# TengdaHan/DPC

Hardware: AMD Instinct MI355X
Metric: clips/sec (train step, B x8x3x5xHxW) (higher is better)
Workload: dtype bf16; 1 GPU; cfg2: resnet18 2d3d, img_dim 128, seq_len 5, num_seq 8, pred_step 3, batch 128/GPU, full train step (fwd+CE/top-k+bwd+all-reduce+Adam); global_batch=128, parallelism=dp1, init=reference init, random, launch=hipGraph replay, streams=2

## Files before the change

### dpc_amd/csrc/bn.hip

```cpp
#include "dpc_rt.h"
#include "../../include/dpc_hip.h"
#include <stdlib.h>

static inline unsigned grid_for(long long n, int block = 256, int cap = 8192) {
    long long g = (n + block - 1) / block;
    if (g < 1) g = 1;
    if (g > cap) g = cap;
    return (unsigned)g;
}

constexpr int FIN_THREADS = 256;
__device__ __forceinline__ void partial_rows_sum(const float* partials, int rows, int C, double& s1, double& s2, double (*red)[4][32]) {
    const int tid = threadIdx.x, q = tid & 7, rl = tid >> 3;
    const int c0 = blockIdx.x * 32 + 4 * q;
    double a[4] = {0.0, 0.0, 0.0, 0.0}, b[4] = {0.0, 0.0, 0.0, 0.0};
    if ((C & 3) == 0 && ((uintptr_t)partials & 15) == 0) {
        if (c0 < C) {
            int r = rl;
            for (; r + 96 < rows; r += 128) {
                f32x4 x[4], y[4];
                DPC_UNROLL
                for (int k = 0; k < 4; ++k) {
                    x[k] = *(const f32x4*)(partials + ((long long)(r + 32 * k) * 2 + 0) * C + c0);
                    y[k] = *(const f32x4*)(partials + ((long long)(r + 32 * k) * 2 + 1) * C + c0);
                }
                DPC_UNROLL
                for (int e = 0; e < 4; ++e) {
                    a[e] += ((double)x[0][e] + (double)x[1][e]) + ((double)x[2][e] + (double)x[3][e]);
                    b[e] += ((double)y[0][e] + (double)y[1][e]) + ((double)y[2][e] + (double)y[3][e]);
                }
            }
            for (; r < rows; r += 32) {
                const f32x4 x = *(const f32x4*)(partials + ((long long)r * 2 + 0) * C + c0);
                const f32x4 y = *(const f32x4*)(partials + ((long long)r * 2 + 1) * C + c0);
                DPC_UNROLL
                for (int e = 0; e < 4; ++e) { a[e] += (double)x[e]; b[e] += (double)y[e]; }
            }
        }
    } else {
        for (int r = rl; r < rows; r += 32)
            DPC_UNROLL
            for (int e = 0; e < 4; ++e)
                if (c0 + e < C) {
                    a[e] += (double)partials[((long long)r * 2 + 0) * C + c0 + e];
                    b[e] += (double)partials[((long long)r * 2 + 1) * C + c0 + e];
                }
    }
    DPC_UNROLL
    for (int m = 8; m < 64; m <<= 1)
        DPC_UNROLL
        for (int e = 0; e < 4; ++e) { a[e] += __shfl_xor(a[e], m); b[e] += __shfl_xor(b[e], m); }
    const int wave = tid >> 6;
    if ((tid & 63) < 8)
        DPC_UNROLL
        for (int e = 0; e < 4; ++e) { red[0][wave][4 * q + e] = a[e]; red[1][wave][4 * q + e] = b[e]; }
    __syncthreads();
    s1 = 0.0; s2 = 0.0;
    if (tid < 32)
        for (int w = 0; w < 4; ++w) { s1 += red[0][w][tid]; s2 += red[1][w][tid]; }
}

__global__ __launch_bounds__(FIN_THREADS) void bn_finalize_kernel(const float* partials, int rows, int C, double count, const float* gamma,
                                   const float* beta, float eps, float* mean, float* invstd, float* scale, float* shift) {
    __shared__ double red[2][4][32];
    const int c = blockIdx.x * 32 + (int)threadIdx.x;
    double s1, s2;
    partial_rows_sum(partials, rows, C, s1, s2, red);
    if (threadIdx.x >= 32 || c >= C) return;
    const double m = s1 / count;
    double var = s2 / count - m * m;
    if (var < 0.0) var = 0.0;
    const double is = 1.0 / sqrt(var + (double)eps);
    mean[c] = (float)m;
    invstd[c] = (float)is;
    const float sc = gamma[c] * (float)is;
    scale[c] = sc;
    shift[c] = beta[c] - (float)m * sc;
}

extern "C" int dpc_bn_finalize(const float* partials, int32_t rows, int32_t C, double count, const float* gamma,
                               const float* beta, float eps, float* mean, float* invstd, float* scale, float* shift,
                               dpc_stream_t stream_) {
    hipStream_t stream = (hipStream_t)stream_;
    if (!partials || rows <= 0 || C <= 0 || count <= 0 || !gamma || !beta || !mean || !invstd || !scale || !shift) return DPC_ERR_ARG;
    DPC_LAUNCH(bn_finalize_kernel, dim3((C + 31) / 32), dim3(FIN_THREADS), stream, partials, rows, C, count, gamma, beta, eps, mean, invstd, scale, shift);
// ... 120 lines not shown
                for (int e = 0; e < E; ++e) {
                    float v = unit_get<T>(xv[u], e) * sc[e] + sh[e];
                    if (res) v += unit_get<T>(rv[u], e) * rs[e] + rb[e];
                    if (relu) v = v > 0.f ? v : 0.f;
                    ov[e] = v;
                }
                const u32x4 o = unit_pack<T>(ov);
                st16<NT>(y, i + u * 256, o);
                if (mask) {
                    DPC_UNROLL
                    for (int e = 0; e < E; ++e) bits |= (unit_get<T>(o, e) > 0.f ? 1u : 0u) << e;
                    mask[i + u * 256] = (uint8_t)bits;
                }
            }
        }
    }
    for (; i < se; i += 256) {
        if (!FIXED) {
            const int c0 = (int)((i * E) % C);
            DPC_UNROLL
            for (int e = 0; e < E; ++e) {
                sc[e] = scale[c0 + e]; sh[e] = shift[c0 + e];
                rs[e] = rscale ? rscale[c0 + e] : 1.f; rb[e] = rscale ? rshift[c0 + e] : 0.f;
            }
        }
        const u32x4 xv = ld16<NT>(x, i);
        u32x4 rv = {0u, 0u, 0u, 0u};
        if (res) rv = ld16<NT>(res, i);
        float ov[E];
        unsigned bits = 0;
        DPC_UNROLL
        for (int e = 0; e < E; ++e) {
            float v = unit_get<T>(xv, e) * sc[e] + sh[e];
            if (res) v += unit_get<T>(rv, e) * rs[e] + rb[e];
            if (relu) v = v > 0.f ? v : 0.f;
            ov[e] = v;
        }
        const u32x4 o = unit_pack<T>(ov);
        st16<NT>(y, i, o);
        if (mask) {
            DPC_UNROLL
            for (int e = 0; e < E; ++e) bits |= (unit_get<T>(o, e) > 0.f ? 1u : 0u) << e;
            mask[i] = (uint8_t)bits;
        }
    }
}

extern "C" int dpc_bn_apply(const void* x, void* y, int32_t dtype, int64_t rows, int32_t C, const float* scale,
                            const float* shift, const void* res, const float* rscale, const float* rshift, int32_t relu,
                            uint8_t* mask, dpc_stream_t stream_) {
    hipStream_t stream = (hipStream_t)stream_;
    if (!x || !y || rows <= 0 || C <= 0 || !scale || !shift) return DPC_ERR_ARG;
    const int E = dtype == DPC_BF16 ? 8 : 4;
    if (C % E) return DPC_ERR_UNSUPPORTED;
    const long long units = rows * C / E;
    const bool fixed = (256 * E) % C == 0;
    static const int rev_on = getenv("DPC_BN_APPLY_REV") ? atoi(getenv("DPC_BN_APPLY_REV")) : 0;
    const int rev = rev_on && bn_streaming(units) ? 1 : 0;
    if (rev && (dtype == DPC_F32 || dtype == DPC_BF16)) dpc_plan_detail("rev");
    if (dtype == DPC_F32) {
        if (fixed) {
            if (bn_streaming(units)) { DPC_LAUNCH((bn_apply_kernel<float, true, true>), dim3(grid_for(units)), dim3(256), stream, (const float*)x, (float*)y, units, C, scale, shift, (const float*)res, rscale, rshift, relu, mask, rev); } else { DPC_LAUNCH((bn_apply_kernel<float, true, false>), dim3(grid_for(units)), dim3(256), stream, (const float*)x, (float*)y, units, C, scale, shift, (const float*)res, rscale, rshift, relu, mask, rev); }
        } else {
            if (bn_streaming(units)) { DPC_LAUNCH((bn_apply_kernel<float, false, true>), dim3(grid_for(units)), dim3(256), stream, (const float*)x, (float*)y, units, C, scale, shift, (const float*)res, rscale, rshift, relu, mask, rev); } else { DPC_LAUNCH((bn_apply_kernel<float, false, false>), dim3(grid_for(units)), dim3(256), stream, (const float*)x, (float*)y, units, C, scale, shift, (const float*)res, rscale, rshift, relu, mask, rev); }
        }
    } else if (dtype == DPC_BF16) {
        if (fixed) {
            const bool nt = bn_streaming(units);
            const int un = nt ? bn_unroll() : bn_small_unroll();
            const unsigned grid = grid_for((units + un - 1) / un, 256, nt ? (un > 1 ? bn_unroll_grid() : 8192) : bn_small_grid(512));
#define DPC_BN_GO(NTV, UV) DPC_LAUNCH((bn_apply_kernel<bf16_t, true, NTV, UV>), dim3(grid), dim3(256), stream, (const bf16_t*)x, (bf16_t*)y, units, C, scale, shift, (const bf16_t*)res, rscale, rshift, relu, mask, rev)
            if (nt) { if (un == 4) DPC_BN_GO(true, 4); else if (un == 2) DPC_BN_GO(true, 2); else DPC_BN_GO(true, 1); }
            else { if (un == 4) DPC_BN_GO(false, 4); else if (un == 2) DPC_BN_GO(false, 2); else DPC_BN_GO(false, 1); }
#undef DPC_BN_GO
        } else {
            if (bn_streaming(units)) { DPC_LAUNCH((bn_apply_kernel<bf16_t, false, true>), dim3(grid_for(units)), dim3(256), stream, (const bf16_t*)x, (bf16_t*)y, units, C, scale, shift, (const bf16_t*)res, rscale, rshift, relu, mask, rev); } else { DPC_LAUNCH((bn_apply_kernel<bf16_t, false, false>), dim3(grid_for(units)), dim3(256), stream, (const bf16_t*)x, (bf16_t*)y, units, C, scale, shift, (const bf16_t*)res, rscale, rshift, relu, mask, rev); }
        }
    } else {
        return DPC_ERR_ARG;
    }
    return dpc_launch_status();
}

template <class T, bool NT, int U = 1>
__global__ __launch_bounds__(256) void bn_bwd_reduce_kernel(const T* dy, const T* y, const uint8_t* mask, const T* x, long long rows, int C,
                                                            const float* mean, const float* invstd, int relu,
                                                            float* partials, long long rows_per_block) {
    constexpr int E = Elt<T>::PER16;
    __shared__ float red[2][256 * E];
    const int upr = C / E;
    const int rpi = 256 / upr;
    const int tid = threadIdx.x;
    const int cu = tid % upr, rr = tid / upr;
    float a1[E], a2[E], mu[E], is[E];
    DPC_UNROLL
    for (int e = 0; e < E; ++e) { a1[e] = 0.f; a2[e] = 0.f; }
    const bool active = rr < rpi;
    if (active) {
        DPC_UNROLL
        for (int e = 0; e < E; ++e) { mu[e] = mean[cu * E + e]; is[e] = invstd[cu * E + e]; }
        const long long r_begin = (long long)blockIdx.x * rows_per_block;
        long long r_end = r_begin + rows_per_block;
        if (r_end > rows) r_end = rows;
        long long r = r_begin + rr;
        if constexpr (U > 1) {
            if (!relu || mask) {
                for (; r + (long long)(U - 1) * rpi < r_end; r += (long long)U * rpi) {
                    u32x4 dv[U], xv[U];
                    unsigned bits[U];
                    DPC_UNROLL
                    for (int u = 0; u < U; ++u) dv[u] = ld16<NT>(dy, (r + (long long)u * rpi) * upr + cu);
                    DPC_UNROLL
                    for (int u = 0; u < U; ++u) xv[u] = ld16<NT>(x, (r + (long long)u * rpi) * upr + cu);
                    DPC_UNROLL
                    for (int u = 0; u < U; ++u) bits[u] = relu ? (unsigned)mask[(r + (long long)u * rpi) * upr + cu] : ~0u;
                    DPC_UNROLL
                    for (int u = 0; u < U; ++u)
                        DPC_UNROLL
                        for (int e = 0; e < E; ++e) {
                            float dz = unit_get<T>(dv[u], e);
                            if (!((bits[u] >> e) & 1u)) dz = 0.f;
                            const float xh = (unit_get<T>(xv[u], e) - mu[e]) * is[e];
                            a1[e] += dz;
                            a2[e] += dz * xh;
                        }
                }
            }
        }
        for (; r < r_end; r += rpi) {
            const long long ui = r * upr + cu;
            const u32x4 dv = ld16<NT>(dy, ui);
            const u32x4 xv = ld16<NT>(x, ui);
            unsigned bits = ~0u;
            if (relu) bits = mask ? (unsigned)mask[ui] : sign_bits<T>(((const u32x4*)y)[ui]);
            DPC_UNROLL
            for (int e = 0; e < E; ++e) {
                float dz = unit_get<T>(dv, e);
                if (!((bits >> e) & 1u)) dz = 0.f;
                const float xh = (unit_get<T>(xv, e) - mu[e]) * is[e];
                a1[e] += dz;
                a2[e] += dz * xh;
            }
        }
    }
    DPC_UNROLL
    for (int e = 0; e < E; ++e) {
        red[0][tid * E + e] = a1[e];
        red[1][tid * E + e] = a2[e];
    }
    __syncthreads();
    if (tid < C) {
        const int cu2 = tid / E, e2 = tid % E;
        float s1 = 0.f, s2 = 0.f;
        for (int g = 0; g < rpi; ++g) {
            const int t2 = g * upr + cu2;
            s1 += red[0][t2 * E + e2];
            s2 += red[1][t2 * E + e2];
        }
        partials[((long long)blockIdx.x * 2 + 0) * C + tid] = s1;
        partials[((long long)blockIdx.x * 2 + 1) * C + tid] = s2;
    }
}

static int bn_bwd_blocks(long long rows, int C, int E, long long* rows_per_block) {
    const int rpi = 256 / (C / E);
    long long per = (long long)rpi * 16;
    long long blocks = (rows + per - 1) / per;
    if (blocks > 1024) {
        blocks = 1024;
        per = (rows + blocks - 1) / blocks;
        per = (per + rpi - 1) / rpi * rpi;
        blocks = (rows + per - 1) / per;
    }
    *rows_per_block = per;
    return (int)blocks;
}

extern "C" int dpc_bn_bwd_reduce(const void* dy, const void* y, const uint8_t* mask, const void* x, int32_t dtype, int64_t rows, int32_t C,
                                 const float* mean, const float* invstd, int32_t relu, float* partials, int32_t* prow,
                                 dpc_stream_t stream_) {
    hipStream_t stream = (hipStream_t)stream_;
    if (rows <= 0 || C <= 0) return DPC_ERR_ARG;
    const int E = dtype == DPC_BF16 ? 8 : 4;
    if (C % E || C / E > 256 || C > 256) return DPC_ERR_UNSUPPORTED;
    long long rpb;
    const int blocks = bn_bwd_blocks(rows, C, E, &rpb);
    if (prow) *prow = blocks;
    if (!partials) return DPC_OK;
    if (!dy || !x || !mean || !invstd || (relu && !y && !mask)) return DPC_ERR_ARG;
    if (dtype == DPC_F32) {
        if (bn_streaming((long long)rows * C / E)) { DPC_LAUNCH((bn_bwd_reduce_kernel<float, true>), dim3(blocks), dim3(256), stream, (const float*)dy, (const float*)y, mask, (const float*)x, (long long)rows, C, mean, invstd, relu, partials, rpb); } else { DPC_LAUNCH((bn_bwd_reduce_kernel<float, false>), dim3(blocks), dim3(256), stream, (const float*)dy, (const float*)y, mask, (const float*)x, (long long)rows, C, mean, invstd, relu, partials, rpb); }
    } else if (dtype == DPC_BF16) {
        const bool nt = bn_streaming((long long)rows * C / E);
        const int un = nt ? bn_unroll() : bn_small_unroll();
#define DPC_BN_GO(NTV, UV) DPC_LAUNCH((bn_bwd_reduce_kernel<bf16_t, NTV, UV>), dim3(blocks), dim3(256), stream, (const bf16_t*)dy, (const bf16_t*)y, mask, (const bf16_t*)x, (long long)rows, C, mean, invstd, relu, partials, rpb)
        if (nt) { if (un > 1) DPC_BN_GO(true, 4); else DPC_BN_GO(true, 1); }
        else { if (un > 1) DPC_BN_GO(false, 4); else DPC_BN_GO(false, 1); }
#undef DPC_BN_GO
    } else {
        return DPC_ERR_ARG;
    }
    return dpc_launch_status();
}

__global__ __launch_bounds__(FIN_THREADS) void bn_bwd_finalize_kernel(const float* partials, int prow, int C, double count, float* dgamma, float* dbeta, float* coef) {
    __shared__ double red[2][4][32];
    const int c = blockIdx.x * 32 + (int)threadIdx.x;
    double s1, s2;
    partial_rows_sum(partials, prow, C, s1, s2, red);
    if (threadIdx.x >= 32 || c >= C) return;
    dbeta[c] = (float)s1;
    dgamma[c] = (float)s2;
    coef[c] = (float)(s1 / count);
    coef[C + c] = (float)(s2 / count);
}

extern "C" int dpc_bn_bwd_finalize(const float* partials, int32_t prow, int32_t C, double count, float* dgamma,
                                   float* dbeta, float* coef, dpc_stream_t stream_) {
    hipStream_t stream = (hipStream_t)stream_;
    if (!partials || prow <= 0 || C <= 0 || count <= 0 || !dgamma || !dbeta || !coef) return DPC_ERR_ARG;
    DPC_LAUNCH(bn_bwd_finalize_kernel, dim3((C + 31) / 32), dim3(FIN_THREADS), stream, partials, prow, C, count, dgamma, dbeta, coef);
    return dpc_launch_status();
}

template <class T, bool FIXED, bool NT, int U = 1>
__global__ void bn_bwd_apply_kernel(const T* dy, const T* y, const uint8_t* mask, const T* x, long long units, int C, const float* mean,
                                    const float* invstd, const float* gamma, const float* coef, int relu, T* dx, T* dzout) {
    constexpr int E = Elt<T>::PER16;
    float mu[E], is[E], ga[E], c1[E], c2[E];
    if (FIXED) {
        const int c0 = (int)((threadIdx.x * E) % C);
        DPC_UNROLL
        for (int e = 0; e < E; ++e) {
            mu[e] = mean[c0 + e]; is[e] = invstd[c0 + e]; ga[e] = gamma[c0 + e] * is[e];
            c1[e] = coef[c0 + e]; c2[e] = coef[C + c0 + e];
        }
    }
    const long long span = (units + (long long)gridDim.x * 256 - 1) / ((long long)gridDim.x * 256) * 256;
    const long long sb = (long long)(gridDim.x - 1 - blockIdx.x) * span;
    const long long se = sb + span < units ? sb + span : units;
    long long i = sb + threadIdx.x;
    if constexpr (FIXED && U > 1) {
        if (!relu || mask) {
            for (; i + (U - 1) * 256 < se; i += 256 * U) {
                u32x4 dv[U], xv[U];
                unsigned bits[U];
                DPC_UNROLL
                for (int u = 0; u < U; ++u) dv[u] = ld16<NT>(dy, i + u * 256);
                DPC_UNROLL
                for (int u = 0; u < U; ++u) xv[u] = ld16<NT>(x, i + u * 256);
                DPC_UNROLL
                for (int u = 0; u < U; ++u) bits[u] = ~0u;
                if (relu) {
                    DPC_UNROLL
                    for (int u = 0; u < U; ++u) bits[u] = (unsigned)mask[i + u * 256];
                }
                DPC_UNROLL
                for (int u = 0; u < U; ++u) {
                    float ov[E], oz[E];
                    DPC_UNROLL
                    for (int e = 0; e < E; ++e) {
                        float dz = unit_get<T>(dv[u], e);
                        if (!((bits[u] >> e) & 1u)) dz = 0.f;
                        const float xh = (unit_get<T>(xv[u], e) - mu[e]) * is[e];
                        ov[e] = ga[e] * (dz - c1[e] - xh * c2[e]);
                        oz[e] = dz;
                    }
                    st16<NT>(dx, i + u * 256, unit_pack<T>(ov));
                    if (dzout) st16<NT>(dzout, i + u * 256, unit_pack<T>(oz));
                }
            }
        }
// ... 61 lines not shown
```

### dpc_amd/csrc/dpc_rt.h

```cpp
#pragma once
#include <stdint.h>
#include <utility>

int dpc_reserved_cus();
static inline int dpc_persistent_grid(int base) {
    int g = base - dpc_reserved_cus();
    if (g < 8) g = 8;
    return base >= 8 ? (g & ~7) : base;
}

extern thread_local int dpc_tls_plan_only;
void dpc_plan_note(const char* kernel_expr);
void dpc_plan_detail(const char* fmt, ...);

#ifdef DPC_SIMT_EMU
#include "simt_emu.h"
#define DPC_LAUNCH(kernel, grid, block, stream, ...)                                   \
    do {                                                                               \
        dpc_plan_note(#kernel);                                                        \
        if (!dpc_tls_plan_only) simt::launch((grid), (block), [=]() { (kernel)(__VA_ARGS__); }); \
    } while (0)
#define DPC_LAUNCH_DYN(kernel, grid, block, lds, stream, ...)                          \
    do {                                                                               \
        dpc_plan_note(#kernel);                                                        \
// ... 318 lines not shown
__device__ __forceinline__ void lds_wait0_5(u32x4&, u32x4&, u32x4&, u32x4&, u32x4&) {}
__device__ __forceinline__ void lds_wait0_4x2(u32x2&, u32x2&, u32x2&, u32x2&) {}
__device__ __forceinline__ void lds_wait0_6x2(u32x2&, u32x2&, u32x2&, u32x2&, u32x2&, u32x2&) {}
#else
__device__ __forceinline__ void lds_read_b64_raw(u32x2& d, const unsigned char* p) {
    const uint32_t a = (uint32_t)(uintptr_t)(__attribute__((address_space(3))) const unsigned char*)p;
    asm volatile("ds_read_b64 %0, %1" : "=&v"(d) : "v"(a) : "memory");
}
__device__ __forceinline__ void lds_read_b128_raw(u32x4& d, const unsigned char* p) { lds_read_b128_async(d, p); }
__device__ __forceinline__ void lds_write_b128_raw(unsigned char* p, const u32x4& v) {
    const uint32_t a = (uint32_t)(uintptr_t)(__attribute__((address_space(3))) unsigned char*)p;
    asm volatile("ds_write_b128 %0, %1" ::"v"(a), "v"(v) : "memory");
}
__device__ __forceinline__ void lds_read_tr16_raw(u32x2& d, const unsigned char* p) {
    const uint32_t a = (uint32_t)(uintptr_t)(__attribute__((address_space(3))) const unsigned char*)p;
    asm volatile("ds_read_b64_tr_b16 %0, %1" : "=&v"(d) : "v"(a) : "memory");
}
__device__ __forceinline__ void lds_wait0_5(u32x4& a, u32x4& b, u32x4& c, u32x4& d, u32x4& e) {
    asm volatile("s_waitcnt lgkmcnt(0)" : "+v"(a), "+v"(b), "+v"(c), "+v"(d), "+v"(e)::"memory");
}
__device__ __forceinline__ void lds_wait0_4x2(u32x2& a, u32x2& b, u32x2& c, u32x2& d) {
    asm volatile("s_waitcnt lgkmcnt(0)" : "+v"(a), "+v"(b), "+v"(c), "+v"(d)::"memory");
}
__device__ __forceinline__ void lds_wait0_6x2(u32x2& a, u32x2& b, u32x2& c, u32x2& d, u32x2& e, u32x2& f) {
    asm volatile("s_waitcnt lgkmcnt(0)" : "+v"(a), "+v"(b), "+v"(c), "+v"(d), "+v"(e), "+v"(f)::"memory");
}
#endif
__device__ __forceinline__ void lds_wait_tie_n(int n, u32x4& a, u32x4& b) {
    if (n >= 6) lds_wait_tie<6>(a, b);
    else if (n == 4) lds_wait_tie<4>(a, b);
    else if (n == 2) lds_wait_tie<2>(a, b);
    else lds_wait_tie<0>(a, b);
}



template <int N> __device__ __forceinline__ void wait_vmcnt() {
#ifndef DPC_SIMT_EMU
    asm volatile("s_waitcnt vmcnt(%0)" ::"n"(N) : "memory");
#else
    simt::dma_wait(N);
#endif
}
__device__ __forceinline__ void vm_note_stores(int n) {
#ifdef DPC_SIMT_EMU
    simt::dma_note_stores(n);
#else
    (void)n;
#endif
}

__device__ __forceinline__ void wait_vmcnt_upto(int n) {
    switch (n) {
        case 0: wait_vmcnt<0>(); break;
        case 1: wait_vmcnt<1>(); break;
        case 2: wait_vmcnt<2>(); break;
        case 3: wait_vmcnt<3>(); break;
        case 4: wait_vmcnt<4>(); break;
        case 5: wait_vmcnt<5>(); break;
        case 6: wait_vmcnt<6>(); break;
        case 7: wait_vmcnt<7>(); break;
        case 8: wait_vmcnt<8>(); break;
        case 9: wait_vmcnt<9>(); break;
        case 10: wait_vmcnt<10>(); break;
        case 11: wait_vmcnt<11>(); break;
        case 12: wait_vmcnt<12>(); break;
        case 13: wait_vmcnt<13>(); break;
        case 14: wait_vmcnt<14>(); break;
        case 15: wait_vmcnt<15>(); break;
        case 16: case 17: wait_vmcnt<16>(); break;
        case 18: case 19: wait_vmcnt<18>(); break;
        case 20: case 21: wait_vmcnt<20>(); break;
        case 22: case 23: wait_vmcnt<22>(); break;
        default: if (n >= 24) wait_vmcnt<24>(); else wait_vmcnt<0>(); break;
    }
}

template <class F, int... Is> __device__ __forceinline__ void static_for_impl(F&& f, std::integer_sequence<int, Is...>) {
    (f(std::integral_constant<int, Is>{}), ...);
}
template <int N, class F> __device__ __forceinline__ void static_for(F&& f) {
    static_for_impl(static_cast<F&&>(f), std::make_integer_sequence<int, N>{});
}
```

### dpc_amd/csrc/pool.hip

```cpp
#include "dpc_rt.h"
#include "../../include/dpc_hip.h"

static inline unsigned grid_for(long long n, int block = 256, int cap = 16384) {
    long long g = (n + block - 1) / block;
    if (g < 1) g = 1;
    if (g > cap) g = cap;
    return (unsigned)g;
}

template <class T>
__global__ void bn_relu_maxpool_fwd_kernel(const T* x, int NT, int H, int W, int C, int Ho, int Wo,
                                           const float* scale, const float* shift, T* y, uint8_t* argmax, int rev) {
    constexpr int E = Elt<T>::PER16;
    const int upr = C / E;
    const long long units = (long long)NT * Ho * Wo * upr;
    unsigned blk = blockIdx.x;
    if ((gridDim.x & 7u) == 0u) blk = (blk & 7u) * (gridDim.x >> 3) + (blk >> 3);
    const long long stride = (long long)gridDim.x * blockDim.x, first = (long long)blk * blockDim.x + threadIdx.x;
    const long long nsweep = first < units ? (units - 1 - first) / stride + 1 : 0;
    for (long long k = 0; k < nsweep; ++k) {
        const long long i = first + (rev ? nsweep - 1 - k : k) * stride;
        const unsigned pidx = (unsigned)(i / upr);
        const int cu = (int)(i - (long long)pidx * upr);
        const unsigned q1 = pidx / (unsigned)Wo;
// ... 180 lines not shown
__global__ __launch_bounds__(256) void pool_bn_bwd_apply_kernel(const T* dy, const uint8_t* argmax, const T* x, int NT, int H, int W, int C,
                                                                int Ho, int Wo, const float* mean, const float* invstd, const float* gamma,
                                                                const float* coef, T* dx, long long quads_per_block) {
    constexpr int E = Elt<T>::PER16;
    const int upr = C / E, rpi = 256 / upr;
    const int tid = threadIdx.x, cu = tid % upr, rr = tid / upr;
    if (rr >= rpi) return;
    const int Qh = (H + 1) / 2, Qw = (W + 1) / 2;
    const long long quads = (long long)NT * Qh * Qw;
    float mu[E], is[E], ga[E], c1[E], c2[E];
    DPC_UNROLL
    for (int e = 0; e < E; ++e) {
        const int c = cu * E + e;
        mu[e] = mean[c]; is[e] = invstd[c]; ga[e] = gamma[c] * is[e]; c1[e] = coef[c]; c2[e] = coef[C + c];
    }
    const long long q_begin = (long long)blockIdx.x * quads_per_block;
    long long q_end = q_begin + quads_per_block;
    if (q_end > quads) q_end = quads;
    for (unsigned q = (unsigned)(q_begin + rr); q < (unsigned)q_end; q += (unsigned)rpi) {
        const unsigned q1 = q / (unsigned)Qw;
        const int b = (int)(q - q1 * (unsigned)Qw);
        const unsigned nt_ = q1 / (unsigned)Qh;
        const int a = (int)(q1 - nt_ * (unsigned)Qh), nt = (int)nt_;
        float g[2][2][E];
        uint32_t am[2][2][2];
        DPC_UNROLL
        for (int i = 0; i < 2; ++i)
            DPC_UNROLL
            for (int j = 0; j < 2; ++j) {
                const bool ok = a + i < Ho && b + j < Wo;
                const long long ui = (long long)((unsigned)((nt * Ho + a + i) * Wo + b + j)) * upr + cu;
                u32x4 gv = {0u, 0u, 0u, 0u};
                am[i][j][0] = 0x09090909u; am[i][j][1] = 0x09090909u;
                if (ok) {
                    gv = ((const u32x4*)dy)[ui];
                    if (E == 8) {
                        const u32x2 t = *(const u32x2*)(argmax + ui * E);
                        am[i][j][0] = t[0]; am[i][j][1] = t[1];
                    } else {
                        am[i][j][0] = *(const uint32_t*)(argmax + ui * E);
                    }
                }
                DPC_UNROLL
                for (int e = 0; e < E; ++e) g[i][j][e] = unit_get<T>(gv, e);
            }
        DPC_UNROLL
        for (int di = 0; di < 2; ++di)
            DPC_UNROLL
            for (int dj = 0; dj < 2; ++dj) {
                const int h = 2 * a + di, w = 2 * b + dj;
                if (h >= H || w >= W) continue;
                float dz[E];
                DPC_UNROLL
                for (int e = 0; e < E; ++e) dz[e] = 0.f;
                DPC_UNROLL
                for (int i = 0; i < 2; ++i)
                    DPC_UNROLL
                    for (int j = 0; j < 2; ++j) {
                        const int kh = di + 1 - 2 * i, kw = dj + 1 - 2 * j;
                        if (kh < 0 || kh > 2 || kw < 0 || kw > 2) continue;
                        const int want = kh * 3 + kw;
                        DPC_UNROLL
                        for (int e = 0; e < E; ++e)
                            if ((int)((am[i][j][e >> 2] >> (8 * (e & 3))) & 0xffu) == want) dz[e] += g[i][j][e];
                    }
                const long long ui = (long long)((unsigned)((nt * H + h) * W + w)) * upr + cu;
                const u32x4 xv = ((const u32x4*)x)[ui];
                float ov[E];
                DPC_UNROLL
                for (int e = 0; e < E; ++e) {
                    const float xh = (unit_get<T>(xv, e) - mu[e]) * is[e];
                    ov[e] = ga[e] * (dz[e] - c1[e] - xh * c2[e]);
                }
                ((u32x4*)dx)[ui] = unit_pack<T>(ov);
            }
    }
}

template <class T>
__global__ __launch_bounds__(256) void pooled_bn_bwd_reduce_kernel(const T* dy, const uint8_t* argmax, const T* ypool, long long rows,
                                                                   int C, const float* gamma, const float* beta, float* partials,
                                                                   long long rows_per_block) {
    constexpr int E = Elt<T>::PER16;
    __shared__ float red[2][256 * E];
    const int upr = C / E, rpi = 256 / upr;
    const int tid = threadIdx.x, cu = tid % upr, rr = tid / upr;
    float a1[E], a2[E], be[E], ig[E];
    DPC_UNROLL
    for (int e = 0; e < E; ++e) { a1[e] = 0.f; a2[e] = 0.f; }
    if (rr < rpi) {
        DPC_UNROLL
        for (int e = 0; e < E; ++e) {
            const float gmm = gamma[cu * E + e];
            be[e] = beta[cu * E + e];
            ig[e] = gmm != 0.f ? 1.f / gmm : 0.f;
        }
        const long long r_begin = (long long)blockIdx.x * rows_per_block;
        long long r_end = r_begin + rows_per_block;
        if (r_end > rows) r_end = rows;
        for (long long r = r_begin + rr; r < r_end; r += rpi) {
            const long long ui = r * upr + cu;
            const u32x4 gv = ((const u32x4*)dy)[ui];
            const u32x4 yv = ((const u32x4*)ypool)[ui];
            uint32_t amw[2] = {0u, 0u};
            if (E == 8) {
                const u32x2 t = *(const u32x2*)(argmax + ui * E);
                amw[0] = t[0]; amw[1] = t[1];
            } else {
                amw[0] = *(const uint32_t*)(argmax + ui * E);
            }
            DPC_UNROLL
            for (int e = 0; e < E; ++e) {
                const bool valid = ((amw[e >> 2] >> (8 * (e & 3))) & 0xffu) < 9u;
                const float dz = valid ? unit_get<T>(gv, e) : 0.f;
                a1[e] += dz;
                a2[e] += dz * (unit_get<T>(yv, e) - be[e]) * ig[e];
            }
        }
    }
    DPC_UNROLL
    for (int e = 0; e < E; ++e) { red[0][tid * E + e] = a1[e]; red[1][tid * E + e] = a2[e]; }
    __syncthreads();
    if (tid < C) {
        const int cu2 = tid / E, e2 = tid % E;
        float s1 = 0.f, s2 = 0.f;
        for (int g = 0; g < rpi; ++g) {
            s1 += red[0][(g * upr + cu2) * E + e2];
            s2 += red[1][(g * upr + cu2) * E + e2];
        }
        partials[((long long)blockIdx.x * 2 + 0) * C + tid] = s1;
        partials[((long long)blockIdx.x * 2 + 1) * C + tid] = s2;
    }
}

static int pool_bwd_blocks(long long rows, int C, int E, long long* rows_per_block) {
    const int rpi = 256 / (C / E);
    long long per = (long long)rpi * 16;
    long long blocks = (rows + per - 1) / per;
    if (blocks > 1024) {
        blocks = 1024;
        per = (rows + blocks - 1) / blocks;
        per = (per + rpi - 1) / rpi * rpi;
        blocks = (rows + per - 1) / per;
    }
    *rows_per_block = per;
    return (int)blocks;
}

extern "C" int dpc_pool_bn_bwd_reduce(const void* dy, const uint8_t* argmax, const void* x, int32_t dtype, int32_t NT, int32_t H,
                                      int32_t W, int32_t C, const float* mean, const float* invstd, float* partials, int32_t* prow,
                                      dpc_stream_t stream_) {
    hipStream_t stream = (hipStream_t)stream_;
    if (NT <= 0 || H <= 0 || W <= 0 || C <= 0) return DPC_ERR_ARG;
    const int E = dtype == DPC_BF16 ? 8 : 4;
    if (C % E || C > 256) return DPC_ERR_UNSUPPORTED;
    long long rpb;
    const int blocks = pool_bwd_blocks((long long)NT * H * W, C, E, &rpb);
    if (prow) *prow = blocks;
    if (!partials) return DPC_OK;
    if (!dy || !argmax || !x || !mean || !invstd) return DPC_ERR_ARG;
    const int Ho = (H - 1) / 2 + 1, Wo = (W - 1) / 2 + 1;
    if (dtype == DPC_F32) {
        DPC_LAUNCH((pool_bn_bwd_reduce_kernel<float>), dim3(blocks), dim3(256), stream, (const float*)dy, argmax, (const float*)x, NT, H, W, C, Ho, Wo, mean, invstd, partials, rpb);
    } else if (dtype == DPC_BF16) {
        DPC_LAUNCH((pool_bn_bwd_reduce_kernel<bf16_t>), dim3(blocks), dim3(256), stream, (const bf16_t*)dy, argmax, (const bf16_t*)x, NT, H, W, C, Ho, Wo, mean, invstd, partials, rpb);
    } else {
        return DPC_ERR_ARG;
    }
    return dpc_launch_status();
}

extern "C" int dpc_pooled_bn_bwd_reduce(const void* dy, const uint8_t* argmax, const void* ypool, int32_t dtype, int64_t rows,
                                        int32_t C, const float* gamma, const float* beta, float* partials, int32_t* prow,
                                        dpc_stream_t stream_) {
    hipStream_t stream = (hipStream_t)stream_;
    if (rows <= 0 || C <= 0) return DPC_ERR_ARG;
    const int E = dtype == DPC_BF16 ? 8 : 4;
    if (C % E || C > 256) return DPC_ERR_UNSUPPORTED;
    long long rpb;
    const int blocks = pool_bwd_blocks(rows, C, E, &rpb);
    if (prow) *prow = blocks;
    if (!partials) return DPC_OK;
    if (!dy || !argmax || !ypool || !gamma || !beta) return DPC_ERR_ARG;
    if (dtype == DPC_F32) {
        DPC_LAUNCH((pooled_bn_bwd_reduce_kernel<float>), dim3(blocks), dim3(256), stream, (const float*)dy, argmax, (const float*)ypool, (long long)rows, C, gamma, beta, partials, rpb);
    } else if (dtype == DPC_BF16) {
        DPC_LAUNCH((pooled_bn_bwd_reduce_kernel<bf16_t>), dim3(blocks), dim3(256), stream, (const bf16_t*)dy, argmax, (const bf16_t*)ypool, (long long)rows, C, gamma, beta, partials, rpb);
    } else {
        return DPC_ERR_ARG;
    }
    return dpc_launch_status();
}

extern "C" int dpc_pool_bn_bwd_apply(const void* dy, const uint8_t* argmax, const void* x, int32_t dtype, int32_t NT, int32_t H,
                                     int32_t W, int32_t C, const float* mean, const float* invstd, const float* gamma,
                                     const float* coef, void* dx, dpc_stream_t stream_) {
    hipStream_t stream = (hipStream_t)stream_;
    if (!dy || !argmax || !x || !dx || !mean || !invstd || !gamma || !coef || NT <= 0 || H <= 0 || W <= 0 || C <= 0) return DPC_ERR_ARG;
    const int E = dtype == DPC_BF16 ? 8 : 4;
    if (C % E) return DPC_ERR_UNSUPPORTED;
    if (C > 256) return DPC_ERR_UNSUPPORTED;
    const int Ho = (H - 1) / 2 + 1, Wo = (W - 1) / 2 + 1;
    const int rpi = 256 / (C / E);
    const long long rows = (long long)NT * ((H + 1) / 2) * ((W + 1) / 2);
    long long blocks = (rows + (long long)rpi * 4 - 1) / ((long long)rpi * 4);
    if (blocks > 16384) blocks = 16384;
    long long rpb = (rows + blocks - 1) / blocks;
    rpb = (rpb + rpi - 1) / rpi * rpi;
    blocks = (rows + rpb - 1) / rpb;
    if (dtype == DPC_F32) {
        DPC_LAUNCH((pool_bn_bwd_apply_kernel<float>), dim3((unsigned)blocks), dim3(256), stream, (const float*)dy, argmax, (const float*)x, NT, H, W, C, Ho, Wo, mean, invstd, gamma, coef, (float*)dx, rpb);
    } else if (dtype == DPC_BF16) {
        DPC_LAUNCH((pool_bn_bwd_apply_kernel<bf16_t>), dim3((unsigned)blocks), dim3(256), stream, (const bf16_t*)dy, argmax, (const bf16_t*)x, NT, H, W, C, Ho, Wo, mean, invstd, gamma, coef, (bf16_t*)dx, rpb);
    } else {
        return DPC_ERR_ARG;
// ... 128 lines not shown
```

Measured before the change: 5067 clips/s.

## Shrink BN backward reduce LDS via wave-shuffle row-group sum and 32-bit offsets

Replaces the per-thread LDS staging of partial sums in the BN and pooled-BN backward reduce kernels with a wave-shuffle reduction that hands off through a small 2x256 float LDS buffer, wave by wave. This cuts shared memory use so more blocks fit per CU, and sets launch bounds to 5 blocks. The row loop now uses 32-bit unit offsets from precomputed base pointers, specializes the unrolled loop on whether a mask gate applies, and adds scheduling fences. A guard rejects cases whose offsets would overflow. The serialized per-wave syncs add latency, and the selective non-contracted multiply changes rounding for some lanes.

```diff
diff --git a/dpc_amd/csrc/bn.hip b/dpc_amd/csrc/bn.hip
--- a/dpc_amd/csrc/bn.hip
+++ b/dpc_amd/csrc/bn.hip
@@ -1,6 +1,7 @@
 #include "dpc_rt.h"
 #include "../../include/dpc_hip.h"
 #include <stdlib.h>
+#include <type_traits>
 
 static inline unsigned grid_for(long long n, int block = 256, int cap = 8192) {
     long long g = (n + block - 1) / block;
@@ -287,12 +288,18 @@
     return dpc_launch_status();
 }
 
+__device__ __forceinline__ float mul_rounded(float a, float b) {
+#ifndef DPC_SIMT_EMU
+#pragma clang fp contract(off)
+#endif
+    return a * b;
+}
 template <class T, bool NT, int U = 1>
-__global__ __launch_bounds__(256) void bn_bwd_reduce_kernel(const T* dy, const T* y, const uint8_t* mask, const T* x, long long rows, int C,
+__global__ __launch_bounds__(256, 5) void bn_bwd_reduce_kernel(const T* dy, const T* y, const uint8_t* mask, const T* x, long long rows, int C,
                                                             const float* mean, const float* invstd, int relu,
                                                             float* partials, long long rows_per_block) {
     constexpr int E = Elt<T>::PER16;
-    __shared__ float red[2][256 * E];
+    __shared__ float hand[2 * 256];
     const int upr = C / E;
     const int rpi = 256 / upr;
     const int tid = threadIdx.x;
@@ -307,37 +314,47 @@
         const long long r_begin = (long long)blockIdx.x * rows_per_block;
         long long r_end = r_begin + rows_per_block;
         if (r_end > rows) r_end = rows;
-        long long r = r_begin + rr;
+        const long long ub = r_begin * upr;
+        const char* pdy = (const char*)dy + ub * 16;
+        const char* px = (const char*)x + ub * 16;
+        const uint8_t* pm = mask ? mask + ub : nullptr;
+        const unsigned nu = (unsigned)((r_end - r_begin) * upr), st = (unsigned)(rpi * upr);
+        unsigned off = (unsigned)tid;
         if constexpr (U > 1) {
-            if (!relu || mask) {
-                for (; r + (long long)(U - 1) * rpi < r_end; r += (long long)U * rpi) {
+            auto trips = [&](auto gated) {
+                for (; off + (U - 1) * st < nu; off += U * st) {
                     u32x4 dv[U], xv[U];
                     unsigned bits[U];
                     DPC_UNROLL
-                    for (int u = 0; u < U; ++u) dv[u] = ld16<NT>(dy, (r + (long long)u * rpi) * upr + cu);
-                    DPC_UNROLL
-                    for (int u = 0; u < U; ++u) xv[u] = ld16<NT>(x, (r + (long long)u * rpi) * upr + cu);
-                    DPC_UNROLL
-                    for (int u = 0; u < U; ++u) bits[u] = relu ? (unsigned)mask[(r + (long long)u * rpi) * upr + cu] : ~0u;
-                    DPC_UNROLL
-                    for (int u = 0; u < U; ++u)
+                    for (int u = 0; u < U; ++u) dv[u] = ld16<NT>(pdy + (off + u * st) * 16u, 0);
+                    DPC_UNROLL
+                    for (int u = 0; u < U; ++u) xv[u] = ld16<NT>(px + (off + u * st) * 16u, 0);
+                    DPC_UNROLL
+                    for (int u = 0; u < U; ++u) bits[u] = decltype(gated)::value ? (unsigned)pm[off + u * st] : ~0u;
+                    DPC_UNROLL
+                    for (int u = 0; u < U; ++u) {
+                        sched_fence();
                         DPC_UNROLL
                         for (int e = 0; e < E; ++e) {
                             float dz = unit_get<T>(dv[u], e);
                             if (!((bits[u] >> e) & 1u)) dz = 0.f;
                             const float xh = (unit_get<T>(xv[u], e) - mu[e]) * is[e];
                             a1[e] += dz;
-                            a2[e] += dz * xh;
+                            if (E == 8 && e >= 6) a2[e] += mul_rounded(dz, xh);
+                            else a2[e] += dz * xh;
                         }
-                }
-            }
-        }
-        for (; r < r_end; r += rpi) {
-            const long long ui = r * upr + cu;
-            const u32x4 dv = ld16<NT>(dy, ui);
-            const u32x4 xv = ld16<NT>(x, ui);
+                    }
+                    sched_fence();
+                }
+            };
+            if (!relu) trips(std::false_type{});
+            else if (mask) trips(std::true_type{});
+        }
+        for (; off < nu; off += st) {
+            const u32x4 dv = ld16<NT>(pdy + off * 16u, 0);
+            const u32x4 xv = ld16<NT>(px + off * 16u, 0);
             unsigned bits = ~0u;
-            if (relu) bits = mask ? (unsigned)mask[ui] : sign_bits<T>(((const u32x4*)y)[ui]);
+            if (relu) bits = mask ? (unsigned)pm[off] : sign_bits<T>(((const u32x4*)y)[ub + off]);
             DPC_UNROLL
             for (int e = 0; e < E; ++e) {
                 float dz = unit_get<T>(dv, e);
@@ -348,23 +365,7 @@
             }
         }
     }
-    DPC_UNROLL
-    for (int e = 0; e < E; ++e) {
-        red[0][tid * E + e] = a1[e];
-        red[1][tid * E + e] = a2[e];
-    }
-    __syncthreads();
-    if (tid < C) {
-        const int cu2 = tid / E, e2 = tid % E;
-        float s1 = 0.f, s2 = 0.f;
-        for (int g = 0; g < rpi; ++g) {
-            const int t2 = g * upr + cu2;
-            s1 += red[0][t2 * E + e2];
-            s2 += red[1][t2 * E + e2];
-        }
-        partials[((long long)blockIdx.x * 2 + 0) * C + tid] = s1;
-        partials[((long long)blockIdx.x * 2 + 1) * C + tid] = s2;
-    }
+    row_groups_sum<E>(a1, a2, upr, rpi, C, hand, partials + (long long)blockIdx.x * 2 * C);
 }
 
 static int bn_bwd_blocks(long long rows, int C, int E, long long* rows_per_block) {
@@ -393,6 +394,7 @@
     if (prow) *prow = blocks;
     if (!partials) return DPC_OK;
     if (!dy || !x || !mean || !invstd || (relu && !y && !mask)) return DPC_ERR_ARG;
+    if (rpb * (C / E) >= (1ll << 28)) return DPC_ERR_UNSUPPORTED;
     if (dtype == DPC_F32) {
         if (bn_streaming((long long)rows * C / E)) { DPC_LAUNCH((bn_bwd_reduce_kernel<float, true>), dim3(blocks), dim3(256), stream, (const float*)dy, (const float*)y, mask, (const float*)x, (long long)rows, C, mean, invstd, relu, partials, rpb); } else { DPC_LAUNCH((bn_bwd_reduce_kernel<float, false>), dim3(blocks), dim3(256), stream, (const float*)dy, (const float*)y, mask, (const float*)x, (long long)rows, C, mean, invstd, relu, partials, rpb); }
     } else if (dtype == DPC_BF16) {
diff --git a/dpc_amd/csrc/dpc_rt.h b/dpc_amd/csrc/dpc_rt.h
--- a/dpc_amd/csrc/dpc_rt.h
+++ b/dpc_amd/csrc/dpc_rt.h
@@ -424,3 +424,37 @@
 template <int N, class F> __device__ __forceinline__ void static_for(F&& f) {
     static_for_impl(static_cast<F&&>(f), std::make_integer_sequence<int, N>{});
 }
+
+template <int E>
+__device__ __forceinline__ void row_groups_sum(const float (&a1)[E], const float (&a2)[E], int upr, int rpi, int C, float* hand, float* out) {
+    const int tid = threadIdx.x, lane = tid & 63, wave = tid >> 6;
+    const int nact = rpi * upr;
+    const bool carrier = lane < upr;
+    int l0 = (carrier ? lane : 0) - (wave * 64) % upr;
+    if (l0 < 0) l0 += upr;
+    float s1[E], s2[E];
+    DPC_UNROLL
+    for (int w = 0; w < 4; ++w) {
+        if (wave == w) {
+            DPC_UNROLL
+            for (int e = 0; e < E; ++e) {
+                s1[e] = w == 0 || !carrier ? 0.f : hand[lane * E + e];
+                s2[e] = w == 0 || !carrier ? 0.f : hand[C + lane * E + e];
+            }
+            for (int src = l0, k = 0; k * upr < 64; ++k, src += upr) {
+                const bool ok = carrier && src < 64 && w * 64 + src < nact;
+                DPC_UNROLL
+                for (int e = 0; e < E; ++e) {
+                    const float v1 = __shfl(a1[e], src & 63), v2 = __shfl(a2[e], src & 63);
+                    if (ok) { s1[e] += v1; s2[e] += v2; }
+                }
+            }
+            if (carrier) {
+                float* dst = w == 3 ? out : hand;
+                DPC_UNROLL
+                for (int e = 0; e < E; ++e) { dst[lane * E + e] = s1[e]; dst[C + lane * E + e] = s2[e]; }
+            }
+        }
+        if (w < 3) __syncthreads();
+    }
+}
diff --git a/dpc_amd/csrc/pool.hip b/dpc_amd/csrc/pool.hip
--- a/dpc_amd/csrc/pool.hip
+++ b/dpc_amd/csrc/pool.hip
@@ -286,7 +286,7 @@
                                                                    int C, const float* gamma, const float* beta, float* partials,
                                                                    long long rows_per_block) {
     constexpr int E = Elt<T>::PER16;
-    __shared__ float red[2][256 * E];
+    __shared__ float hand[2 * 256];
     const int upr = C / E, rpi = 256 / upr;
     const int tid = threadIdx.x, cu = tid % upr, rr = tid / upr;
     float a1[E], a2[E], be[E], ig[E];
@@ -322,19 +322,7 @@
             }
         }
     }
-    DPC_UNROLL
-    for (int e = 0; e < E; ++e) { red[0][tid * E + e] = a1[e]; red[1][tid * E + e] = a2[e]; }
-    __syncthreads();
-    if (tid < C) {
-        const int cu2 = tid / E, e2 = tid % E;
-        float s1 = 0.f, s2 = 0.f;
-        for (int g = 0; g < rpi; ++g) {
-            s1 += red[0][(g * upr + cu2) * E + e2];
-            s2 += red[1][(g * upr + cu2) * E + e2];
-        }
-        partials[((long long)blockIdx.x * 2 + 0) * C + tid] = s1;
-        partials[((long long)blockIdx.x * 2 + 1) * C + tid] = s2;
-    }
+    row_groups_sum<E>(a1, a2, upr, rpi, C, hand, partials + (long long)blockIdx.x * 2 * C);
 }
 
 static int pool_bwd_blocks(long long rows, int C, int E, long long* rows_per_block) {
```

Result: no change. 5083 clips/s (median of 6 runs) (+0.3%).
